# soedinglab/spacedust

Measured on AMD Instinct MI355X. Metric: clustersearch throughput (genome-pairs/s; SW GCUPS alongside), higher is better.
Workload: dtype int16

## Files before the change

### include/spacedust_gpu.h

```cpp
#ifndef SPACEDUST_GPU_H
#define SPACEDUST_GPU_H

#include <stddef.h>
#include <stdint.h>

#ifdef __cplusplus
extern "C" {
#endif

enum {
    SD_OK = 0,
    SD_ENODEVICE = -1,
    SD_EHIP = -2,
    SD_EINVAL = -3,
    SD_ENOMEM = -4,
    SD_EUNSUPPORTED = -5,
    SD_EMISMATCH = -6
};

typedef struct sd_ctx sd_ctx;
typedef struct sd_seqset sd_seqset;
typedef struct sd_target sd_target;

int sd_ctx_create(int device, sd_ctx **out);
// ... 59 lines not shown
                                    uint32_t nPairs, const uint32_t *pairQ, const uint32_t *pairT, const uint16_t *pairDiag,
                                    const uint8_t *isIdentity, float seqIdThr, int32_t alnLenThr, uint32_t *outIdx, sd_sw_result *out,
                                    uint32_t *nOut, char *btPool, uint64_t btCap, uint64_t *btUsed);

int sd_sw_align_alt_batch(sd_ctx *ctx, const sd_sw_params *par, const sd_seqset *queries, const sd_seqset *targets, uint32_t nSeeds,
                          const uint32_t *seedQ, const uint32_t *seedT, const int32_t *tStart, const int32_t *tEnd,
                          const uint8_t *isIdentity, uint32_t maxAlt, float seqIdThr, int32_t alnLenThr, int32_t seqIdMode,
                          sd_sw_result *out, uint32_t *outCount, char *btPool, uint64_t btCap, uint64_t *btUsed);
int sd_sw_alt_last_stats(sd_ctx *ctx, uint64_t *groups, uint64_t *seedRounds, uint64_t *bytesCopied);

int sd_sw_set_cigar_pool(sd_ctx *ctx, int on);
int sd_sw_download_bytes(sd_ctx *ctx, uint64_t *recordBytes, uint64_t *poolBytes);

int sd_sw_set_narrow_final(sd_ctx *ctx, int on);
int sd_sw_set_shared_start(sd_ctx *ctx, int on);

int sd_selftest_sort_pairs(sd_ctx *ctx, const uint32_t *keys, const uint32_t *vals, uint32_t n, int beginBit, int endBit, uint32_t *outKeys,
                           uint32_t *outVals);
int sd_selftest_scan(sd_ctx *ctx, const uint32_t *in, uint32_t n, uint64_t *exclusiveSum, uint32_t *runningMax);
int sd_selftest_score_class(int kernel , int32_t n, int32_t tL, int shared, int32_t wideRowLimit,
                            uint32_t *klass, char *scope, size_t cap);
int sd_selftest_r2p_weights(sd_ctx *ctx, uint32_t nTasks, const uint32_t *nRows, const uint32_t *L, const uint8_t *cells, float *freq,
                            float *eff);
struct sd_kmermatch_params_s;
int sd_selftest_kmermatch_records(sd_ctx *ctx, const struct sd_kmermatch_params_s *par, uint64_t nSeq, const uint8_t *residues,
                                  const uint64_t *offsets, const uint32_t *keys, const uint8_t *letterMap21, uint64_t recCap,
                                  uint32_t *seqConsidered, uint32_t *seqThreshold, uint32_t *seqExcess, uint64_t *recOff, uint64_t *recKey,
                                  uint32_t *recId, uint32_t *recLen, uint32_t *recPos, uint64_t *stats);

int sd_sw_align_batch_hostpath(sd_ctx *ctx, const sd_sw_params *par, const sd_seqset *queries, const sd_seqset *targets,
// ... 430 lines not shown
```

### spacedust_amd/_lib.py

```python
import ctypes as C
import os

import numpy as np

HERE = os.path.dirname(os.path.abspath(__file__))
LIB_PATH = os.path.join(HERE, 'libsdgpu.so')

_vp = C.c_void_p


SD_OK, SD_ENODEVICE, SD_EHIP, SD_EINVAL, SD_ENOMEM, SD_EUNSUPPORTED, SD_EMISMATCH = 0, -1, -2, -3, -4, -5, -6


class SdError(RuntimeError):
    pass


class SwParams(C.Structure):
    _fields_ = [('gapOpen', C.c_int32), ('gapExtend', C.c_int32), ('matrix', C.c_int8 * 441), ('covMode', C.c_int32),
                ('covThr', C.c_float), ('evalThr', C.c_double), ('swMode', C.c_int32), ('dbResidues', C.c_uint64)]


class SwResult(C.Structure):
    _fields_ = [('score', C.c_int32), ('qStart', C.c_int32), ('qEnd', C.c_int32), ('tStart', C.c_int32),
# ... 223 lines not shown
        'sd_search_result_arrays': (C.c_int, [_vp] + [_vp] * 12),
        'sd_search_result_write_tsv': (C.c_int, [_vp, C.c_char_p, C.c_char_p, _vp, C.c_char_p, _vp, C.c_char_p, _vp, C.c_char_p, _vp,
                                                 C.c_int, C.c_int, C.c_uint64, C.POINTER(C.c_uint64), C.POINTER(C.c_uint64)]),
        'sd_search_result_records': (C.c_int, [_vp, _vp, C.c_uint64, C.POINTER(C.c_uint64)]),
        'sd_agg_records': (C.c_int, [_vp] * 7 + [_vp, C.c_uint64, C.POINTER(C.c_uint64)]),
        'sd_records_check': (C.c_int, [_vp, C.c_uint64, C.c_uint32, C.c_uint32, C.c_uint32, C.c_uint32, C.POINTER(C.c_uint64), C.POINTER(C.c_uint64)]),
        'sd_records_write_tsv': (C.c_int, [_vp, C.c_uint64, C.c_char_p, C.c_int, C.c_uint64, C.c_char_p, _vp, C.c_char_p, _vp, C.c_char_p, _vp,
                                           C.c_char_p, _vp, C.c_int, C.POINTER(C.c_uint64), C.POINTER(C.c_uint64)]),
        'sd_search_result_destroy': (None, [_vp]),
        'sd_search_stats': (C.c_int, [_vp, _vp, _vp]),
        'sd_search_download_bytes': (C.c_int, [_vp, C.POINTER(C.c_uint64), C.POINTER(C.c_uint64)]),
        'sd_sw_set_cigar_pool': (C.c_int, [_vp, C.c_int]),
        'sd_sw_download_bytes': (C.c_int, [_vp, C.POINTER(C.c_uint64), C.POINTER(C.c_uint64)]),
        'sd_sw_set_narrow_final': (C.c_int, [_vp, C.c_int]),
        'sd_sw_set_shared_start': (C.c_int, [_vp, C.c_int]),
        'sd_r2p_create': (C.c_int, [C.POINTER(_vp)]),
        'sd_r2p_destroy': (None, [_vp]),
        'sd_r2p_batch': (C.c_int, [_vp, C.POINTER(R2pParams), C.c_uint32] + [_vp] * 12),
        'sd_r2p_batch_device': (C.c_int, [_vp, _vp, C.POINTER(R2pParams), C.c_uint32] + [_vp] * 12),
        'sd_selftest_r2p_weights': (C.c_int, [_vp, C.c_uint32, _vp, _vp, _vp, _vp, _vp]),
        'sd_selftest_score_class': (C.c_int, [C.c_int, C.c_int32, C.c_int32, C.c_int, C.c_int32, C.POINTER(C.c_uint32), C.c_char_p, C.c_size_t]),
        'sd_shard_query_sets': (C.c_int, [_vp, C.c_uint32, C.c_uint32, C.c_uint32, _vp, C.POINTER(C.c_uint32)]),
        'sd_comm_unique_id': (C.c_int, [C.c_char_p]),
        'sd_comm_init': (C.c_int, [C.c_int, C.c_int, C.c_int, C.c_char_p, C.POINTER(_vp)]),
        'sd_comm_destroy': (None, [_vp]),
        'sd_comm_host_buffer': (C.c_int, [_vp, C.c_int, C.c_uint64, C.POINTER(_vp)]),
        'sd_comm_last_error': (C.c_char_p, [_vp]),
        'sd_search_set_records_sink': (C.c_int, [_vp, _vp, _vp]),
        'sd_gather_stream_begin': (C.c_int, [_vp, C.c_int, C.c_uint32, _vp, C.c_uint32, _vp, C.c_uint64, C.c_int, C.POINTER(_vp)]),
        'sd_gather_stream_end': (C.c_int, [_vp, _vp, _vp, C.POINTER(C.c_uint64)]),
# ... 62 lines not shown
```

### spacedust_amd/api.py

```python
import ctypes as C

import numpy as np

from . import _lib
from .cpus import effective_cpus
from ._lib import SdError, ptr


def _check(ctx, rc, what):
    if rc != 0:
        msg = ''
        if ctx is not None:
            msg = _lib.load().sd_last_error(ctx).decode(errors='replace')
        raise SdError('%s failed (%d): %s' % (what, rc, msg))


class Host:

    def __init__(self, threads=0):
        import os
        self.L = _lib.load()
        self.threads = threads or effective_cpus()
        h = C.c_void_p()
        _check(None, self.L.sd_host_create(self.threads, C.byref(h)), 'sd_host_create')
# ... 444 lines not shown
        out = np.zeros(len(hq), _lib.RESCORE_DTYPE)
        _check(self.h, self.L.sd_rescore_diagonal_batch(self.h, C.byref(par), queries.h, targets.h, len(hq), ptr(hq), ptr(ht), ptr(hd),
                                                        ptr(out)), 'sd_rescore_diagonal_batch')
        return out

    def set_cigar_pool(self, on=True):
        _check(self.h, self.L.sd_sw_set_cigar_pool(self.h, 1 if on else 0), 'sd_sw_set_cigar_pool')
        self._cigar_pool = bool(on)

    def set_narrow_final(self, on=True):
        _check(self.h, self.L.sd_sw_set_narrow_final(self.h, 1 if on else 0), 'sd_sw_set_narrow_final')

    def set_shared_start(self, on=True):
        _check(self.h, self.L.sd_sw_set_shared_start(self.h, 1 if on else 0), 'sd_sw_set_shared_start')

    def sw_download_bytes(self):
        a, b = C.c_uint64(), C.c_uint64()
        self.L.sd_sw_download_bytes(self.h, C.byref(a), C.byref(b))
        return a.value, b.value

    def sw_cells(self):
        f, r, t = C.c_uint64(), C.c_uint64(), C.c_uint64()
        self.L.sd_sw_last_cells(self.h, C.byref(f), C.byref(r), C.byref(t))
        return f.value, r.value, t.value

    def __del__(self):
        try:
            h, self.h = self.h, None
            if h:
                self.L.sd_ctx_destroy(h)
# ... 511 lines not shown
```

### spacedust_amd/csrc/cli/sd_mod_iter.cpp

```cpp
#include "sd_align_core.h"
#include "sd_cli.h"
#include "sd_pref_core.h"

#include <algorithm>
#include <atomic>
#include <chrono>
#include <climits>
#include <cmath>
#include <condition_variable>
#include <cstdio>
#include <cstdlib>
#include <cstring>
#include <memory>
#include <mutex>
#include <omp.h>
#include <string>
#include <sys/resource.h>
#include <thread>
#include <vector>

namespace sdcli {

namespace {

// ... 43 lines not shown

struct Worker {
    sd_ctx *ctx = nullptr;
    sd_host *host = nullptr;
    sd_r2p *r2p = nullptr;
    int threads = 1;
    QueryChunk Q;
    std::vector<uint8_t> failed;
    AlignChunk C;
    std::vector<uint32_t> mark;
    uint32_t stamp = 0;
    ~Worker() {
        if (r2p) sd_r2p_destroy(r2p);
        if (ctx) sd_sw_set_narrow_final(ctx, 0);
        if (ctx) sd_sw_set_shared_start(ctx, 0);
        if (ctx) sd_ctx_destroy(ctx);
        if (host) sd_host_destroy(host);
    }
};

double quantE(double v) {
    char text[32];
    double back = v;
    sd_host_quantise_3e(v, text, &back);
    return back;
}

int failChunk(ChunkOut &o, int rc, const std::string &what, sd_ctx *ctx) {
    o.rc = rc;
    o.err = what + " failed (" + std::to_string(rc) + ")";
// ... 255 lines not shown
    nWorkers = std::max(1, std::min(nWorkers, 8));
    uint32_t chunkQ = (uint32_t) std::max<long long>(1, a.integer("--iter-chunk-queries", getenv("SD_ITER_CHUNK") ? atoi(getenv("SD_ITER_CHUNK")) : 1500));
    const int perWorker = std::max(1, std::min(threads, (threads * 3 / 2 + nWorkers - 1) / nWorkers));
    std::vector<std::unique_ptr<Worker> > workers;
    for (int w = 0; w < nWorkers; w++) {
        workers.emplace_back(new Worker());
        Worker &W = *workers.back();
        W.threads = perWorker;
        int rc = sd_ctx_create(device, &W.ctx);
        if (rc != SD_OK) return failNoDevice(rc);
        if (sd_host_create(perWorker, &W.host) != SD_OK) return fail("sd_host_create failed");
        if (sd_r2p_create(&W.r2p) != SD_OK) return fail("sd_r2p_create failed");
        if (S.profile) sd_profile_enable(W.ctx, 1);
        sd_sw_set_narrow_final(W.ctx, (getenv("SD_SW_NARROW_FINAL") && atoi(getenv("SD_SW_NARROW_FINAL")) == 0) ? 0 : 1);
        sd_sw_set_shared_start(W.ctx, (getenv("SD_SW_SHARED_START") && atoi(getenv("SD_SW_SHARED_START")) == 0) ? 0 : 1);
    }
    uint64_t indexEntries = 0;
    TargetH seqTarget, profTarget;
    SeqSetH tset;
    {
        sd_ctx *c0 = workers[0]->ctx;
        uint64_t st[2] = {0, 0};
        if (int rc = buildTarget(host.h, c0, S.pfSeq, tdb->residues.data(), tdb->offsets.data(), tdb->n, &seqTarget.t, st)) return rc;
        indexEntries = st[0];
        info(a, "Index table k-mer threshold: %d at k-mer size %d\nIndex statistics\nEntries:          %llu\n", S.pfSeq.kmerThr, S.pfSeq.k,
             (unsigned long long) st[0]);
        if (numIt > 1) {
            if (int rc = buildTarget(host.h, c0, S.pfProf, tdb->residues.data(), tdb->offsets.data(), tdb->n, &profTarget.t, st, std::string(),
                                     "sd_target_build (profile searches)"))
                return rc;
// ... 420 lines not shown
```

### spacedust_amd/csrc/hip/sd_common.h

```cpp
#ifndef SD_COMMON_H
#define SD_COMMON_H

#include <hip/hip_runtime.h>

#include <cstdarg>
#include <cstdint>
#include <cstdio>
#include <cstring>
#include <algorithm>
#include <ctime>
#include <sys/prctl.h>
#include <map>
#include <mutex>
#include <string>
#include <vector>

#include "spacedust_gpu.h"

struct sd_profile_entry {
    double ms = 0.0;
    uint64_t launches = 0;
};

struct sd_ctx {
    int device = 0;
    hipStream_t stream = nullptr;
    std::string lastError;
    bool profiling = false;
    std::map<std::string, sd_profile_entry> profile;
    hipEvent_t evStart = nullptr, evStop = nullptr;
    bool biasTablesUploaded = false;
    hipEvent_t evSync = nullptr;
    uint64_t cellsFwd = 0, cellsRev = 0, cellsTb = 0;
    uint64_t cellsUngapped = 0;
    uint64_t altGroups = 0, altSeedRounds = 0, altBytes = 0;
    const sd_sw_result *alignDevRes = nullptr;
    size_t alignDevResN = 0;
    bool cigarPool = false;
    bool sharedStart = false;
    bool narrowFinal = false;
    uint64_t d2hRecordBytes = 0, d2hPoolBytes = 0;
    struct ExpandState {
        uint64_t nPairs = 0, runsRead = 0, bytesWritten = 0;
        uint32_t nAB = 0;
        const int32_t *abStartA = nullptr, *abStartB = nullptr, *bcStartB = nullptr, *bcStartC = nullptr;
        const uint64_t *abRunOff = nullptr, *bcRowOff = nullptr, *bcRunOff = nullptr, *pairOff = nullptr;
        const uint32_t *abRuns = nullptr, *bcRuns = nullptr, *abCluster = nullptr;
        const sd_expand_result *res = nullptr;
    } expand;
    hipDeviceProp_t prop;
    struct WsEntry { void *p = nullptr; size_t bytes = 0; };
    std::map<std::string, WsEntry> ws;
    std::map<std::string, WsEntry> pinned;
    struct ProfPending { std::string name; hipEvent_t a = nullptr, b = nullptr; };
// ... 343 lines not shown
```

### spacedust_amd/csrc/hip/sd_sw.hip

```cpp
#include "sd_common.h"
#include <unistd.h>


#include <algorithm>
#include <cmath>
#include <cstring>
#include <memory>
#include <omp.h>
#include <numeric>

#include "../host/sd_host.h"
#include "sd_sw_pk.h"

namespace {

using sdpk::SwTask;
using sdpk::NARROW_EXACT;

template <int RT>
__global__ void __launch_bounds__(64)
sw_score_kernel(const SwTask *__restrict__ tasks, uint32_t nTasks, const uint8_t *__restrict__ qRes,
                const int8_t *__restrict__ qBias, const uint8_t *__restrict__ tRes, const int8_t *__restrict__ mat,
                int go, int ge, int32_t *__restrict__ out, uint2 *__restrict__ boundary,
                const uint32_t *__restrict__ order ,
// ... 673 lines not shown
}

using ScoreLaunch = void (*)(sd_ctx *ctx, const SwTask *dTasks, const uint32_t *dOrder, uint32_t n, const sd_seqset *q, const sd_seqset *t,
                             const int8_t *dMat, int go, int ge, int32_t *dOut, uint2 *dBound);

template <int RT, int LW, bool MULTI, bool WIDE, bool SHARED>
void launchScorePk(sd_ctx *ctx, const SwTask *dTasks, const uint32_t *dOrder, uint32_t n, const sd_seqset *q,
                   const sd_seqset *t, const int8_t *dMat, int go, int ge, int32_t *dOut, uint2 *dBound) {
    if (n == 0) return;
    constexpr uint32_t perWave = 2 * (64 / LW);
    dim3 grid((n + perWave - 1) / perWave), block(64);
    hipLaunchKernelGGL((sdpk::sw_score_pk_kernel<RT, LW, MULTI, WIDE, SHARED>), grid, block, 0, ctx->stream, dTasks, n, q->dRes, q->dBias,
                       t->dRes, dMat, go, ge, dOut, dBound, dOrder, (const int8_t *) q->dProf);
}

template <int RT, bool SHARED, bool START = false>
void launchScorePkAligned(sd_ctx *ctx, const SwTask *dTasks, const uint32_t *dOrder, uint32_t n, const sd_seqset *q, const sd_seqset *t,
                          const int8_t *dMat, int go, int ge, int32_t *dOut, uint2 * ) {
    if (n == 0) return;
    constexpr uint32_t perWave = 4;
    dim3 grid((n + perWave - 1) / perWave), block(64);
    hipLaunchKernelGGL((sdpk::sw_score_pk_aligned_kernel<RT, SHARED, START>), grid, block, 0, ctx->stream, dTasks, n, q->dRes, q->dBias, t->dRes,
                       dMat, go, ge, dOut, dOrder, (const int8_t *) q->dProf);
}

template <int RT>
void launchScoreIdx(sd_ctx *ctx, const SwTask *dTasks, const uint32_t *dOrder, uint32_t n, const sd_seqset *q,
                    const sd_seqset *t, const int8_t *dMat, int go, int ge, int32_t *dOut, uint2 *dBound) {
    if (n == 0) return;
    dim3 grid((n + 1) / 2), block(64);
    hipLaunchKernelGGL(sw_score_kernel<RT>, grid, block, 0, ctx->stream, dTasks, n, q->dRes, q->dBias, t->dRes, dMat,
                       go, ge, dOut, dBound, dOrder, (const int8_t *) q->dProf);
}

enum ScoreKernel { SCORE_PK = 0, SCORE_PK_WIDE = 1, SCORE_INT32 = 2, SCORE_PK_START = 3 };
constexpr int START_ROWS_MIN = 129, START_ROWS_MAX = 768;
// ... 746 lines not shown
    }
    need[i] = v;
}
__global__ void __launch_bounds__(256)
k_bound_apply(uint32_t nPairs, SwTask *__restrict__ tasks, const uint64_t *__restrict__ off) {
    const uint32_t i = blockIdx.x * blockDim.x + threadIdx.x;
    if (i >= nPairs) return;
    tasks[i].boundOff = off[i];
}

constexpr uint32_t PAIR_NONE = 0xFFFFFFFFu;
constexpr int PAIR_QUERY_BITS = 17;
__host__ __device__ __forceinline__ bool pairedClass(uint32_t ci, int startOnly) {
    return startOnly ? ci >= FIRST_START_CLASS && ci < N_SCORE_CLASSES : ci < FIRST_INT32_CLASS;
}
__global__ void __launch_bounds__(256)
k_pair_keys(uint32_t n, const uint32_t *__restrict__ keys, const uint32_t *__restrict__ pairQ, uint32_t *__restrict__ key2, int startOnly) {
    const uint32_t i = blockIdx.x * blockDim.x + threadIdx.x;
    if (i >= n) return;
    const uint32_t k = keys[i];
    uint32_t v = k == KEY_INVALID ? 0xFFFFFFFFu : ((k >> 10) << 26) | (pairQ[i] << 9) | ((k & 1023u) >> 1);
    if (startOnly && k != KEY_INVALID && !pairedClass(k >> 10, startOnly)) v = ((k >> 10) << 26) | ((k & 1023u) << 16);
    key2[i] = v;
}
__global__ void __launch_bounds__(256)
k_pair_heads(uint32_t n, const uint32_t *__restrict__ keyS, uint32_t *__restrict__ headPos) {
    const uint32_t p = blockIdx.x * blockDim.x + threadIdx.x;
    if (p >= n) return;
    const bool head = p == 0 || (keyS[p] >> 9) != (keyS[p - 1] >> 9);
    headPos[p] = head ? p : 0u;
}
__global__ void __launch_bounds__(256)
k_pair_leaders(uint32_t n, const uint32_t *__restrict__ keyS, const uint32_t *__restrict__ runStart, uint8_t *__restrict__ leader,
               int startOnly) {
    const uint32_t p = blockIdx.x * blockDim.x + threadIdx.x;
    if (p > n) return;
    uint8_t v = 0;
    if (p < n && pairedClass(keyS[p] >> 26, startOnly)) {
        const uint32_t o = p - runStart[p];
        v = (o & 1u) == 0 ? 1 : 0;
        const bool lastOfRun = p + 1 >= n || (keyS[p + 1] >> 9) != (keyS[p] >> 9);
        const uint32_t pairs = (o + 1 + 1) / 2;
        if (lastOfRun) v += (uint8_t) (pairs & 1u);
    }
    leader[p] = v;
}
__global__ void __launch_bounds__(256)
k_pair_emit(uint32_t n, const uint32_t *__restrict__ keyS, const uint32_t *__restrict__ vals, const uint32_t *__restrict__ runStartOf,
            const uint64_t *__restrict__ pairIdx, uint32_t *__restrict__ order2, int startOnly) {
    const uint32_t p = blockIdx.x * blockDim.x + threadIdx.x;
    if (p >= n || !pairedClass(keyS[p] >> 26, startOnly) || ((p - runStartOf[p]) & 1u)) return;
    const uint64_t w = pairIdx[p];
    order2[2 * w] = vals[p];
    const bool mate = p + 1 < n && (keyS[p + 1] >> 9) == (keyS[p] >> 9);
    order2[2 * w + 1] = mate ? vals[p + 1] : PAIR_NONE;
}
__global__ void k_pair_bounds(const uint32_t *__restrict__ keyS, uint32_t n, const uint64_t *__restrict__ pairIdx,
                              uint32_t *__restrict__ b, int nb) {
// ... 30 lines not shown
                int startOnly = 0 ) {
    const uint32_t *dOrder = w.dOrder;
    const unsigned grid = (nPairs + 255) / 256;
    int rc = SD_OK;
    uint32_t *dOrder2 = nullptr, *dPairBounds = nullptr;
    if (dPairQ) {
        uint32_t *dKey2 = nullptr, *dVals2 = nullptr, *dHead = nullptr, *dRunStart = nullptr;
        uint64_t *dPairIdx = nullptr;
        uint8_t *dLeader = nullptr;
        SD_HIP(ctx, wsGet(ctx, "sp.key2", (size_t) nPairs, &dKey2));
        SD_HIP(ctx, wsGet(ctx, "sp.vals2", (size_t) nPairs, &dVals2));
        SD_HIP(ctx, wsGet(ctx, "sp.head", (size_t) nPairs, &dHead));
        SD_HIP(ctx, wsGet(ctx, "sp.runstart", (size_t) nPairs, &dRunStart));
        SD_HIP(ctx, wsGet(ctx, "sp.leader", (size_t) nPairs + 1, &dLeader));
        SD_HIP(ctx, wsGet(ctx, "sp.pairidx", (size_t) nPairs + 1, &dPairIdx));
        const size_t order2Cap = (size_t) 4 * nPairs + 8;
        SD_HIP(ctx, wsGet(ctx, "sp.order2", order2Cap, &dOrder2));
        SD_HIP(ctx, hipMemsetAsync(dOrder2, 0xFF, order2Cap * sizeof(uint32_t), ctx->stream));
        SD_HIP(ctx, wsGet(ctx, "sp.bounds", 64, &dPairBounds));
        hipLaunchKernelGGL(k_pair_keys, dim3(grid), dim3(256), 0, ctx->stream, nPairs, dKeys, dPairQ, dKey2, startOnly);
        rc = devSortPairs(ctx, dKey2, w.dKeysS, w.dVals, dVals2, nPairs, 32);
        if (rc != SD_OK) return rc;
        dOrder = dVals2;
        hipLaunchKernelGGL(k_pair_heads, dim3(grid), dim3(256), 0, ctx->stream, nPairs, w.dKeysS, dHead);
        rc = devInclusiveMax(ctx, dHead, dRunStart, nPairs);
        if (rc != SD_OK) return rc;
        hipLaunchKernelGGL(k_pair_leaders, dim3((nPairs + 256) / 256), dim3(256), 0, ctx->stream, nPairs, w.dKeysS, dRunStart, dLeader, startOnly);
        rc = devExclusiveScan(ctx, (const uint8_t *) dLeader, dPairIdx, (size_t) nPairs + 1);
        if (rc != SD_OK) return rc;
        hipLaunchKernelGGL(k_pair_emit, dim3(grid), dim3(256), 0, ctx->stream, nPairs, w.dKeysS, dVals2, dRunStart, dPairIdx, dOrder2, startOnly);
        hipLaunchKernelGGL(k_pair_bounds, dim3(1), dim3(64), 0, ctx->stream, w.dKeysS, nPairs, dPairIdx, dPairBounds,
                           (int) N_SCORE_CLASSES + 1);
        hipLaunchKernelGGL(k_bounds, dim3(1), dim3(64), 0, ctx->stream, w.dKeysS, nPairs, 1u << 26, w.dBounds, (int) N_SCORE_CLASSES + 1);
    } else {
        rc = devSortPairs(ctx, dKeys, w.dKeysS, w.dVals, w.dOrder, nPairs, 16);
        if (rc != SD_OK) return rc;
        hipLaunchKernelGGL(k_bounds, dim3(1), dim3(64), 0, ctx->stream, w.dKeysS, nPairs, 1024u, w.dBounds, (int) N_SCORE_CLASSES + 1);
    }
    hipLaunchKernelGGL(k_bound_need, dim3(grid), dim3(256), 0, ctx->stream, nPairs, w.dTasks, dKeys, w.dScanA);
    SD_HIP(ctx, hipMemsetAsync(w.dScanA + nPairs, 0, sizeof(uint64_t), ctx->stream));
    rc = devExclusiveScan(ctx, w.dScanA, w.dScanB, (size_t) nPairs + 1);
    if (rc != SD_OK) return rc;
// ... 875 lines not shown
int sd_sw_set_cigar_pool(sd_ctx *ctx, int on) {
    if (!ctx) return SD_EINVAL;
    ctx->cigarPool = on != 0;
    return SD_OK;
}

int sd_sw_set_narrow_final(sd_ctx *ctx, int on) {
    if (!ctx) return SD_EINVAL;
    ctx->narrowFinal = on != 0;
    return SD_OK;
}

int sd_sw_set_shared_start(sd_ctx *ctx, int on) {
    if (!ctx) return SD_EINVAL;
    ctx->sharedStart = on != 0;
    return SD_OK;
}

int sd_sw_download_bytes(sd_ctx *ctx, uint64_t *recordBytes, uint64_t *poolBytes) {
    if (!ctx) return SD_EINVAL;
    if (recordBytes) *recordBytes = ctx->d2hRecordBytes;
    if (poolBytes) *poolBytes = ctx->d2hPoolBytes;
    return SD_OK;
}

int sd_sw_align_batch(sd_ctx *ctx, const sd_sw_params *par, const sd_seqset *queries, const sd_seqset *targets,
                      uint32_t nPairs, const uint32_t *pairQ, const uint32_t *pairT, const uint8_t *isIdentity,
                      sd_sw_result *out, char *btPool, uint64_t btCap, uint64_t *btUsed) {
    return alignBatchImpl(ctx, {par, queries, targets, nPairs, pairQ, pairT, isIdentity, out, btPool, btCap, btUsed, nullptr, nullptr, nullptr, nullptr});
}
// ... 308 lines not shown
```

### spacedust_amd/csrc/hip/sd_sw_pk.h

```cpp
#ifndef SD_SW_PK_H
#define SD_SW_PK_H

#include <hip/hip_runtime.h>
#include <cstdint>

namespace sdpk {

struct SwTask {
    uint64_t qOff;
    uint64_t tOff;
    int32_t n;
    int32_t tL;
    int32_t qStep;
    int32_t tStep;
    int32_t segLen;
    uint32_t slot;
    uint64_t boundOff;
};

typedef short s16x2 __attribute__((ext_vector_type(2)));
typedef unsigned short u16x2 __attribute__((ext_vector_type(2)));

__device__ __forceinline__ uint32_t pkMax(uint32_t a, uint32_t b) {
    return __builtin_bit_cast(uint32_t, __builtin_elementwise_max(__builtin_bit_cast(s16x2, a), __builtin_bit_cast(s16x2, b)));
// ... 26 lines not shown
    asm("v_add_u16_sdwa %0, %4, sext(%8) dst_sel:WORD_0 dst_unused:UNUSED_PAD src0_sel:WORD_0 src1_sel:BYTE_0\n\t"
        "v_add_u16_sdwa %1, %5, sext(%8) dst_sel:WORD_0 dst_unused:UNUSED_PAD src0_sel:WORD_0 src1_sel:BYTE_1\n\t"
        "v_add_u16_sdwa %2, %6, sext(%8) dst_sel:WORD_0 dst_unused:UNUSED_PAD src0_sel:WORD_0 src1_sel:BYTE_2\n\t"
        "v_add_u16_sdwa %3, %7, sext(%8) dst_sel:WORD_0 dst_unused:UNUSED_PAD src0_sel:WORD_0 src1_sel:BYTE_3\n\t"
        "v_add_u16_sdwa %0, %4, sext(%9) dst_sel:WORD_1 dst_unused:UNUSED_PRESERVE src0_sel:WORD_1 src1_sel:BYTE_0\n\t"
        "v_add_u16_sdwa %1, %5, sext(%9) dst_sel:WORD_1 dst_unused:UNUSED_PRESERVE src0_sel:WORD_1 src1_sel:BYTE_1\n\t"
        "v_add_u16_sdwa %2, %6, sext(%9) dst_sel:WORD_1 dst_unused:UNUSED_PRESERVE src0_sel:WORD_1 src1_sel:BYTE_2\n\t"
        "v_add_u16_sdwa %3, %7, sext(%9) dst_sel:WORD_1 dst_unused:UNUSED_PRESERVE src0_sel:WORD_1 src1_sel:BYTE_3\n\t"
        "s_nop 0"
        : "=&v"(h0), "=&v"(h1), "=&v"(h2), "=&v"(h3)
        : "v"(d0), "v"(d1), "v"(d2), "v"(d3), "v"(pa), "v"(pb));
}

__device__ __forceinline__ uint32_t dppShr1(uint32_t v) {
    return (uint32_t) __builtin_amdgcn_update_dpp(0, (int) v, 0x138 , 0xf, 0xf, false);
}

template <int LANE>
__device__ __forceinline__ uint32_t writeLane(uint32_t value, uint32_t old) {
    asm("v_writelane_b32 %0, %1, %2" : "+v"(old) : "s"(value), "n"(LANE));
    return old;
}
__device__ __forceinline__ uint32_t readLane(uint32_t v, int lane) {
#if defined(__HIP_DEVICE_COMPILE__)
    return (uint32_t) __builtin_amdgcn_readlane((int) v, lane);
#else
    (void) lane;
    return v;
#endif
}
// ... 267 lines not shown
    uint32_t r;
    asm("v_bfi_b32 %0, %1, %2, %3" : "=v"(r) : "v"(mask), "v"(a), "v"(b));
    return r;
}
__device__ __forceinline__ uint32_t addWord0(uint32_t base, uint32_t packed) {
    uint32_t r;
    asm("v_add_u32_sdwa %0, %1, %2 dst_sel:DWORD dst_unused:UNUSED_PAD src0_sel:DWORD src1_sel:WORD_0" : "=v"(r) : "v"(base), "v"(packed));
    return r;
}
__device__ __forceinline__ uint32_t addWord1(uint32_t base, uint32_t packed) {
    uint32_t r;
    asm("v_add_u32_sdwa %0, %1, %2 dst_sel:DWORD dst_unused:UNUSED_PAD src0_sel:DWORD src1_sel:WORD_1" : "=v"(r) : "v"(base), "v"(packed));
    return r;
}

template <int RT, bool SHARED, bool START = false>
__global__ void __launch_bounds__(64)
sw_score_pk_aligned_kernel(const SwTask *__restrict__ tasks, uint32_t nTasks, const uint8_t *__restrict__ qRes,
                           const int8_t *__restrict__ qBias, const uint8_t *__restrict__ tRes, const int8_t *__restrict__ mat,
                           int go, int ge, int32_t *__restrict__ out, const uint32_t *__restrict__ order,
                           const int8_t *__restrict__ qProf) {
    constexpr int LW = 32;
    constexpr int WORDS = (RT + 3) / 4;
    constexpr int RTP = 4 * WORDS;
    constexpr int PSTRIDE = LW * WORDS;
    constexpr int NGRP = 64 / LW;
    constexpr int NT = 2 * NGRP;
    constexpr uint32_t ROWB = PSTRIDE * 4;
    static_assert(22 * ROWB < 65536, "row offsets travel in 16 bits");
    static_assert(SHARED || !START, "the start-row form has one profile per wavefront");
    __shared__ uint32_t prof[SHARED ? 1 : NT][22][PSTRIDE];
    __shared__ int8_t smat[441];
    for (int i = threadIdx.x; i < 441; i += 64) smat[i] = mat[i];
    __syncthreads();
    const int lane = threadIdx.x & 63, wave = threadIdx.x >> 6;
    const int grp = lane / LW, l = lane % LW;
    SwTask tk[NT];
#pragma unroll
    for (int x = 0; x < NT; x++) {
        const uint32_t id = (blockIdx.x + (uint32_t) wave) * NT + x;
        const uint32_t tid = id < nTasks ? (order ? order[id] : id) : 0xFFFFFFFFu;
        if (tid != 0xFFFFFFFFu) {
            tk[x] = tasks[tid];
        } else {
            tk[x].n = 0; tk[x].tL = 0; tk[x].qOff = 0; tk[x].tOff = 0; tk[x].qStep = 1; tk[x].tStep = 1; tk[x].segLen = START ? 0 : 1;
// ... 8 lines not shown
            B = tk[2 * g + 1];
        }
    const bool haveA = A.n > 0, haveB = B.n > 0;
    if (SHARED && !haveB) {
        B = A;
        B.tL = 0;
    }
    int maxN = 0, maxTL = 0;
#pragma unroll
    for (int x = 0; x < NT; x++) {
        maxN = max(maxN, tk[x].n);
        maxTL = max(maxTL, tk[x].tL);
    }
    const int steps = (maxN > 0 && maxTL > 0) ? maxTL + LW - 1 : 0;
    const uint32_t goP = (uint32_t) go | ((uint32_t) go << 16), geP = (uint32_t) ge | ((uint32_t) ge << 16);
    const int q0 = l * RT;
#pragma unroll
    for (int x = 0; x < (SHARED ? 1 : 2); x++) {
        const SwTask &T = SHARED ? tk[0] : (x ? B : A);
        const int64_t pOff = START ? (int64_t) T.qOff - (int64_t) T.segLen * T.qStep : (int64_t) T.qOff;
        const int pN = START ? T.n + T.segLen : T.n;
        uint32_t *pw = &prof[SHARED ? 0 : 2 * grp + x][0][0] + l * WORDS;
#pragma unroll
        for (int w = 0; w < WORDS; w++) {
            int res[4], cb[4];
            int64_t pidx[4];
            bool valid[4];
#pragma unroll
            for (int b = 0; b < 4; b++) {
                const int qi = q0 + 4 * w + b;
                valid[b] = (4 * w + b < RT) && qi < pN;
                res[b] = 20;
                cb[b] = 0;
                pidx[b] = 0;
                if (valid[b]) {
                    const int64_t idx = pOff + (int64_t) qi * T.qStep;
                    res[b] = qRes[idx];
                    cb[b] = qBias[idx];
                    pidx[b] = idx * 21;
                }
            }
            const int aFirst = SHARED ? wave * NGRP + grp : 0, aStep = SHARED ? NGRP : 1;
            if (qProf) {
                for (int a = aFirst; a < 21; a += aStep) {
                    uint32_t word = 0;
#pragma unroll
// ... 42 lines not shown
            keepA[w] = l != sA ? 0xFFFFFFFFu : (dropA == 4 ? 0u : 0xFFFFFFFFu << (8 * dropA));
            keepB[w] = l != sB ? 0xFFFFFFFFu : (dropB == 4 ? 0u : 0xFFFFFFFFu << (8 * dropB));
        }
    }
    constexpr uint32_t NEUT = (uint32_t) PK_NEUTRAL * ROWB;
    auto loadChunk = [&](int c0) -> uint32_t {
        const int col = c0 + l;
        uint32_t a = PK_NEUTRAL, b = PK_NEUTRAL;
        if (col < A.tL) a = tRes[(int64_t) A.tOff + (int64_t) col * A.tStep];
        if (col < B.tL) b = tRes[(int64_t) B.tOff + (int64_t) col * B.tStep];
        return (a * ROWB) | ((b * ROWB) << 16);
    };
    uint32_t chunk = loadChunk(0);
    uint32_t chunkNext = loadChunk(LW);
    uint32_t T = NEUT | (NEUT << 16);
    T = writeLane<0>(readLane(chunk, 0), T);
    T = writeLane<32>(readLane(chunk, 32), T);
    uint32_t pa[WORDS], pb[WORDS];
    {
        const uint32_t aA = addWord0(baseA, T), aB = addWord1(baseB, T);
#pragma unroll
        for (int w = 0; w < WORDS; w++) {
            pa[w] = ldsWord(aA, w);
            pb[w] = ldsWord(aB, w);
        }
    }
    auto columnStep = [&](const int k, const uint32_t &Tc, const uint32_t (&pac)[WORDS], const uint32_t (&pbc)[WORDS], uint32_t &Tn,
                          uint32_t (&pan)[WORDS], uint32_t (&pbn)[WORDS]) {
        const int i1 = (k + 1) & (LW - 1);
        if (i1 == 0) {
            chunk = chunkNext;
            chunkNext = loadChunk(k + 1 + LW);
        }
        Tn = dppShr1(Tc);
        Tn = writeLane<0>(readLane(chunk, i1), Tn);
        Tn = writeLane<32>(readLane(chunk, 32 + i1), Tn);
        {
            const uint32_t aA = addWord0(baseA, Tn), aB = addWord1(baseB, Tn);
#pragma unroll
            for (int w = 0; w < WORDS; w++) {
                pan[w] = ldsWord(aA, w);
                pbn[w] = ldsWord(aB, w);
            }
        }
        uint32_t inG = dppShr1(outG), inFf = dppShr1(outFf);
        if (START) {
            inG &= handMask;
            inFf &= handMask;
        } else {
            inG = writeLane<32>(0, inG);
            inFf = writeLane<32>(0, inFf);
        }
        uint32_t h[RTP];
#pragma unroll
        for (int w = 0; w < WORDS; w++) {
            const uint32_t d0 = (w == 0) ? prevInG : H[4 * w - 1];
            const uint32_t qa = START ? bfiAsm(keepA[w], pac[w], neutralWord) : pac[w];
            const uint32_t qb = START ? bfiAsm(keepB[w], pbc[w], neutralWord) : pbc[w];
            addProfile4(qa, qb, d0, H[4 * w], H[4 * w + 1], H[4 * w + 2], h[4 * w], h[4 * w + 1], h[4 * w + 2], h[4 * w + 3]);
        }
        prevInG = inG;
        uint32_t Ff = inFf, cm = 0;
#pragma unroll
        for (int r = 0; r < RT; r++) {
            const uint32_t hpre = pkMax(h[r], E[r]);
            const uint32_t g = pkMax(hpre, Ff);
            const uint32_t open = pkSubSat(hpre, goP);
            E[r] = pkMax(pkSubSat(E[r], geP), open);
            Ff = pkMax(pkSubSat(Ff, geP), open);
            H[r] = g;
            const uint32_t code = pkRowCode(g, 31 - r);
            cm = r == 0 ? code : pkMax(cm, code);
        }
        outG = H[RT - 1];
        outFf = Ff;
        const uint32_t t = bestcm | 0x001F001Fu;
        const uint32_t m = pkAshr15(pkSub(t, cm));
        const uint32_t kk = (uint32_t) k | ((uint32_t) k << 16);
        bestcm = bfiAsm(m, cm, bestcm);
        bestcol = bfiAsm(m, kk, bestcol);
    };
    uint32_t T2, pa2[WORDS], pb2[WORDS];
#pragma unroll 1
    for (int k = 0; k < steps; k += 2) {
        columnStep(k, T, pa, pb, T2, pa2, pb2);
        columnStep(k + 1, T2, pa2, pb2, T, pa, pb);
    }
    unsigned long long keyA = 0, keyB = 0;
    {
// ... 32 lines not shown
```

### spacedust_amd/csrc/host/sd_search.cpp

```cpp
#include "sd_host.h"
#include "sd_target_build.h"
#include "spacedust_gpu.h"

#include <algorithm>
#include <chrono>
#include <condition_variable>
#include <cstdio>
#include <cstdlib>
#include <cstring>
#include <deque>
#include <fstream>
#include <functional>
#include <future>
#include <memory>
#include <mutex>
#include <string>
#include <thread>
#include <pthread.h>
#include <vector>

namespace {

double nowSec() {
    return std::chrono::duration<double>(std::chrono::steady_clock::now().time_since_epoch()).count();
// ... 459 lines not shown
            for (sd_ctx *c : al)
                if (c) sd_sw_set_narrow_final(c, 0);
        }
    } narrowFinalMode(s, !(getenv("SD_SW_NARROW_FINAL") && atoi(getenv("SD_SW_NARROW_FINAL")) == 0));
    struct SharedStartMode {
        sd_ctx *al[4];
        explicit SharedStartMode(sd_search *s_, bool on) : al{s_->ctxAl, s_->ctxAl2, s_->ctxAlMore[0], s_->ctxAlMore[1]} {
            for (sd_ctx *c : al)
                if (c) sd_sw_set_shared_start(c, on ? 1 : 0);
        }
        ~SharedStartMode() {
            for (sd_ctx *c : al)
                if (c) sd_sw_set_shared_start(c, 0);
        }
    } sharedStartMode(s, !(getenv("SD_SW_SHARED_START") && atoi(getenv("SD_SW_SHARED_START")) == 0));
    std::vector<uint32_t> qSetSize(Q->nSets, 0);
    if (aggregate)
        for (uint32_t i = 0; i < Q->n; i++)
            if (Q->setId[i] < Q->nSets) qSetSize[Q->setId[i]]++;
    if (aggregate) {
        uint32_t m = 0;
        for (uint32_t v : qSetSize) m = std::max(m, v);
        for (uint32_t v : s->tSetSize) m = std::max(m, v);
        for (uint32_t i = 0; i < Q->n; i++) m = std::max(m, Q->posInSet[i]);
        for (uint32_t i = 0; i < T.n; i++) m = std::max(m, T.posInSet[i]);
        if (s->lgamma.size() < (size_t) m + 8) {
            s->lgamma.resize((size_t) m + 8);
            sd_host_lgamma_table(s->lgamma.data(), (uint32_t) s->lgamma.size());
        }
    }
// ... 586 lines not shown
```

Before: 3044.

## Pack four query-sharing pairs per wavefront using 16-lane DPP-row groups

Adds a group16 mode, on by default, for the shared-profile aligned scoring kernel. For aligned classes up to 448 rows, each 32-lane half-wavefront is split into two 16-lane DPP rows, each handling twice as many rows per lane. A wavefront then processes four pairs sharing one query profile instead of two. Leader padding and order-buffer sizing change so query runs are grouped in multiples of four. The aim is to cut wasted diagonal steps and lane idle time for shorter queries, at the cost of more registers per lane, longer per-lane row loops, and more padding slots.

```diff
diff --git a/include/spacedust_gpu.h b/include/spacedust_gpu.h
--- a/include/spacedust_gpu.h
+++ b/include/spacedust_gpu.h
@@ -97,6 +97,7 @@
 
 int sd_sw_set_narrow_final(sd_ctx *ctx, int on);
 int sd_sw_set_shared_start(sd_ctx *ctx, int on);
+int sd_sw_set_group16(sd_ctx *ctx, int on);
 
 int sd_selftest_sort_pairs(sd_ctx *ctx, const uint32_t *keys, const uint32_t *vals, uint32_t n, int beginBit, int endBit, uint32_t *outKeys,
                            uint32_t *outVals);
diff --git a/spacedust_amd/_lib.py b/spacedust_amd/_lib.py
--- a/spacedust_amd/_lib.py
+++ b/spacedust_amd/_lib.py
@@ -261,6 +261,7 @@
         'sd_sw_download_bytes': (C.c_int, [_vp, C.POINTER(C.c_uint64), C.POINTER(C.c_uint64)]),
         'sd_sw_set_narrow_final': (C.c_int, [_vp, C.c_int]),
         'sd_sw_set_shared_start': (C.c_int, [_vp, C.c_int]),
+        'sd_sw_set_group16': (C.c_int, [_vp, C.c_int]),
         'sd_r2p_create': (C.c_int, [C.POINTER(_vp)]),
         'sd_r2p_destroy': (None, [_vp]),
         'sd_r2p_batch': (C.c_int, [_vp, C.POINTER(R2pParams), C.c_uint32] + [_vp] * 12),
diff --git a/spacedust_amd/api.py b/spacedust_amd/api.py
--- a/spacedust_amd/api.py
+++ b/spacedust_amd/api.py
@@ -482,6 +482,9 @@
     def set_shared_start(self, on=True):
         _check(self.h, self.L.sd_sw_set_shared_start(self.h, 1 if on else 0), 'sd_sw_set_shared_start')
 
+    def set_group16(self, on=True):
+        _check(self.h, self.L.sd_sw_set_group16(self.h, 1 if on else 0), 'sd_sw_set_group16')
+
     def sw_download_bytes(self):
         a, b = C.c_uint64(), C.c_uint64()
         self.L.sd_sw_download_bytes(self.h, C.byref(a), C.byref(b))
diff --git a/spacedust_amd/csrc/cli/sd_mod_iter.cpp b/spacedust_amd/csrc/cli/sd_mod_iter.cpp
--- a/spacedust_amd/csrc/cli/sd_mod_iter.cpp
+++ b/spacedust_amd/csrc/cli/sd_mod_iter.cpp
@@ -81,6 +81,7 @@
         if (r2p) sd_r2p_destroy(r2p);
         if (ctx) sd_sw_set_narrow_final(ctx, 0);
         if (ctx) sd_sw_set_shared_start(ctx, 0);
+        if (ctx) sd_sw_set_group16(ctx, 0);
         if (ctx) sd_ctx_destroy(ctx);
         if (host) sd_host_destroy(host);
     }
@@ -366,6 +367,7 @@
         if (S.profile) sd_profile_enable(W.ctx, 1);
         sd_sw_set_narrow_final(W.ctx, (getenv("SD_SW_NARROW_FINAL") && atoi(getenv("SD_SW_NARROW_FINAL")) == 0) ? 0 : 1);
         sd_sw_set_shared_start(W.ctx, (getenv("SD_SW_SHARED_START") && atoi(getenv("SD_SW_SHARED_START")) == 0) ? 0 : 1);
+        sd_sw_set_group16(W.ctx, (getenv("SD_SW_GROUP16") && atoi(getenv("SD_SW_GROUP16")) == 0) ? 0 : 1);
     }
     uint64_t indexEntries = 0;
     TargetH seqTarget, profTarget;
diff --git a/spacedust_amd/csrc/hip/sd_common.h b/spacedust_amd/csrc/hip/sd_common.h
--- a/spacedust_amd/csrc/hip/sd_common.h
+++ b/spacedust_amd/csrc/hip/sd_common.h
@@ -38,6 +38,7 @@
     size_t alignDevResN = 0;
     bool cigarPool = false;
     bool sharedStart = false;
+    bool group16 = false;
     bool narrowFinal = false;
     uint64_t d2hRecordBytes = 0, d2hPoolBytes = 0;
     struct ExpandState {
diff --git a/spacedust_amd/csrc/hip/sd_sw.hip b/spacedust_amd/csrc/hip/sd_sw.hip
--- a/spacedust_amd/csrc/hip/sd_sw.hip
+++ b/spacedust_amd/csrc/hip/sd_sw.hip
@@ -711,12 +711,23 @@
                        t->dRes, dMat, go, ge, dOut, dBound, dOrder, (const int8_t *) q->dProf);
 }
 
+constexpr int GROUP16_ROWS_MAX = 448;
+constexpr __host__ __device__ uint32_t pairsPerWave(uint32_t ci, int startOnly, int group16);
+constexpr uint32_t alignedClass(int RT) { return (uint32_t) RT - 4; }
+
 template <int RT, bool SHARED, bool START = false>
 void launchScorePkAligned(sd_ctx *ctx, const SwTask *dTasks, const uint32_t *dOrder, uint32_t n, const sd_seqset *q, const sd_seqset *t,
                           const int8_t *dMat, int go, int ge, int32_t *dOut, uint2 * ) {
     if (n == 0) return;
-    constexpr uint32_t perWave = 4;
+    const uint32_t perWave = (SHARED && !START) ? 2 * pairsPerWave(alignedClass(RT), 0, ctx->group16 ? 1 : 0) : 4;
     dim3 grid((n + perWave - 1) / perWave), block(64);
+    if constexpr (SHARED && !START && 32 * RT <= GROUP16_ROWS_MAX) {
+        if (perWave == 8) {
+            hipLaunchKernelGGL((sdpk::sw_score_pk_aligned_kernel<RT, true, false, 16>), grid, block, 0, ctx->stream, dTasks, n, q->dRes, q->dBias,
+                               t->dRes, dMat, go, ge, dOut, dOrder, (const int8_t *) q->dProf);
+            return;
+        }
+    }
     hipLaunchKernelGGL((sdpk::sw_score_pk_aligned_kernel<RT, SHARED, START>), grid, block, 0, ctx->stream, dTasks, n, q->dRes, q->dBias, t->dRes,
                        dMat, go, ge, dOut, dOrder, (const int8_t *) q->dProf);
 }
@@ -1493,6 +1504,12 @@
 __host__ __device__ __forceinline__ bool pairedClass(uint32_t ci, int startOnly) {
     return startOnly ? ci >= FIRST_START_CLASS && ci < N_SCORE_CLASSES : ci < FIRST_INT32_CLASS;
 }
+constexpr __host__ __device__ uint32_t pairsPerWave(uint32_t ci, int startOnly, int group16) {
+    return group16 && !startOnly && ci >= alignedClass(5) && ci <= alignedClass(GROUP16_ROWS_MAX / 32) ? 4u : 2u;
+}
+static_assert(SCORE_CLASSES[alignedClass(5)].form == SCORE_PK && SCORE_CLASSES[alignedClass(5)].rows == 5 * 32 &&
+              SCORE_CLASSES[alignedClass(24)].form == SCORE_PK && SCORE_CLASSES[alignedClass(24)].rows == 24 * 32,
+              "alignedClass: a_seg5 .. a_seg24 are the classes 1 .. 20");
 __global__ void __launch_bounds__(256)
 k_pair_keys(uint32_t n, const uint32_t *__restrict__ keys, const uint32_t *__restrict__ pairQ, uint32_t *__restrict__ key2, int startOnly) {
     const uint32_t i = blockIdx.x * blockDim.x + threadIdx.x;
@@ -1511,7 +1528,7 @@
 }
 __global__ void __launch_bounds__(256)
 k_pair_leaders(uint32_t n, const uint32_t *__restrict__ keyS, const uint32_t *__restrict__ runStart, uint8_t *__restrict__ leader,
-               int startOnly) {
+               int startOnly, int group16) {
     const uint32_t p = blockIdx.x * blockDim.x + threadIdx.x;
     if (p > n) return;
     uint8_t v = 0;
@@ -1520,7 +1537,8 @@
         v = (o & 1u) == 0 ? 1 : 0;
         const bool lastOfRun = p + 1 >= n || (keyS[p + 1] >> 9) != (keyS[p] >> 9);
         const uint32_t pairs = (o + 1 + 1) / 2;
-        if (lastOfRun) v += (uint8_t) (pairs & 1u);
+        const uint32_t ppw = pairsPerWave(keyS[p] >> 26, startOnly, group16);
+        if (lastOfRun) v += (uint8_t) ((ppw - pairs % ppw) % ppw);
     }
     leader[p] = v;
 }
@@ -1581,7 +1599,7 @@
         SD_HIP(ctx, wsGet(ctx, "sp.runstart", (size_t) nPairs, &dRunStart));
         SD_HIP(ctx, wsGet(ctx, "sp.leader", (size_t) nPairs + 1, &dLeader));
         SD_HIP(ctx, wsGet(ctx, "sp.pairidx", (size_t) nPairs + 1, &dPairIdx));
-        const size_t order2Cap = (size_t) 4 * nPairs + 8;
+        const size_t order2Cap = (size_t) 8 * nPairs + 16;
         SD_HIP(ctx, wsGet(ctx, "sp.order2", order2Cap, &dOrder2));
         SD_HIP(ctx, hipMemsetAsync(dOrder2, 0xFF, order2Cap * sizeof(uint32_t), ctx->stream));
         SD_HIP(ctx, wsGet(ctx, "sp.bounds", 64, &dPairBounds));
@@ -1592,7 +1610,8 @@
         hipLaunchKernelGGL(k_pair_heads, dim3(grid), dim3(256), 0, ctx->stream, nPairs, w.dKeysS, dHead);
         rc = devInclusiveMax(ctx, dHead, dRunStart, nPairs);
         if (rc != SD_OK) return rc;
-        hipLaunchKernelGGL(k_pair_leaders, dim3((nPairs + 256) / 256), dim3(256), 0, ctx->stream, nPairs, w.dKeysS, dRunStart, dLeader, startOnly);
+        hipLaunchKernelGGL(k_pair_leaders, dim3((nPairs + 256) / 256), dim3(256), 0, ctx->stream, nPairs, w.dKeysS, dRunStart, dLeader, startOnly,
+                           ctx->group16 ? 1 : 0);
         rc = devExclusiveScan(ctx, (const uint8_t *) dLeader, dPairIdx, (size_t) nPairs + 1);
         if (rc != SD_OK) return rc;
         hipLaunchKernelGGL(k_pair_emit, dim3(grid), dim3(256), 0, ctx->stream, nPairs, w.dKeysS, dVals2, dRunStart, dPairIdx, dOrder2, startOnly);
@@ -2498,6 +2517,12 @@
 int sd_sw_set_shared_start(sd_ctx *ctx, int on) {
     if (!ctx) return SD_EINVAL;
     ctx->sharedStart = on != 0;
+    return SD_OK;
+}
+
+int sd_sw_set_group16(sd_ctx *ctx, int on) {
+    if (!ctx) return SD_EINVAL;
+    ctx->group16 = on != 0;
     return SD_OK;
 }
 
diff --git a/spacedust_amd/csrc/hip/sd_sw_pk.h b/spacedust_amd/csrc/hip/sd_sw_pk.h
--- a/spacedust_amd/csrc/hip/sd_sw_pk.h
+++ b/spacedust_amd/csrc/hip/sd_sw_pk.h
@@ -64,6 +64,16 @@
 
 __device__ __forceinline__ uint32_t dppShr1(uint32_t v) {
     return (uint32_t) __builtin_amdgcn_update_dpp(0, (int) v, 0x138 , 0xf, 0xf, false);
+}
+
+__device__ __forceinline__ uint32_t dppRowShr1(uint32_t v) {
+    return (uint32_t) __builtin_amdgcn_update_dpp(0, (int) v, 0x111 , 0xf, 0xf, true);
+}
+__device__ __forceinline__ uint32_t dppRowShr1Keep(uint32_t first, uint32_t v) {
+    return (uint32_t) __builtin_amdgcn_update_dpp((int) first, (int) v, 0x111 , 0xf, 0xf, false);
+}
+__device__ __forceinline__ uint32_t dppRowRol1(uint32_t v) {
+    return (uint32_t) __builtin_amdgcn_update_dpp(0, (int) v, 0x12F , 0xf, 0xf, false);
 }
 
 template <int LANE>
@@ -361,21 +371,24 @@
     return r;
 }
 
-template <int RT, bool SHARED, bool START = false>
+template <int RT, bool SHARED, bool START = false, int LW = 32>
 __global__ void __launch_bounds__(64)
 sw_score_pk_aligned_kernel(const SwTask *__restrict__ tasks, uint32_t nTasks, const uint8_t *__restrict__ qRes,
                            const int8_t *__restrict__ qBias, const uint8_t *__restrict__ tRes, const int8_t *__restrict__ mat,
                            int go, int ge, int32_t *__restrict__ out, const uint32_t *__restrict__ order,
                            const int8_t *__restrict__ qProf) {
-    constexpr int LW = 32;
-    constexpr int WORDS = (RT + 3) / 4;
+    constexpr int RTL = RT * (32 / LW);
+    constexpr int WORDS = (RTL + 3) / 4;
     constexpr int RTP = 4 * WORDS;
     constexpr int PSTRIDE = LW * WORDS;
     constexpr int NGRP = 64 / LW;
     constexpr int NT = 2 * NGRP;
     constexpr uint32_t ROWB = PSTRIDE * 4;
+    static_assert(LW == 32 || LW == 16, "a group is half a wavefront or one DPP row");
     static_assert(22 * ROWB < 65536, "row offsets travel in 16 bits");
     static_assert(SHARED || !START, "the start-row form has one profile per wavefront");
+    static_assert(LW == 32 || (SHARED && !START), "16-lane groups: the shared forward form only");
+    static_assert(RTL <= 32, "the row code has five row bits: 16-lane groups end at RT = 16 (512 rows), a_seg17 .. a_seg24 stay on 32 lanes");
     __shared__ uint32_t prof[SHARED ? 1 : NT][22][PSTRIDE];
     __shared__ int8_t smat[441];
     for (int i = threadIdx.x; i < 441; i += 64) smat[i] = mat[i];
@@ -414,7 +427,7 @@
     }
     const int steps = (maxN > 0 && maxTL > 0) ? maxTL + LW - 1 : 0;
     const uint32_t goP = (uint32_t) go | ((uint32_t) go << 16), geP = (uint32_t) ge | ((uint32_t) ge << 16);
-    const int q0 = l * RT;
+    const int q0 = l * RTL;
 #pragma unroll
     for (int x = 0; x < (SHARED ? 1 : 2); x++) {
         const SwTask &T = SHARED ? tk[0] : (x ? B : A);
@@ -429,7 +442,7 @@
 #pragma unroll
             for (int b = 0; b < 4; b++) {
                 const int qi = q0 + 4 * w + b;
-                valid[b] = (4 * w + b < RT) && qi < pN;
+                valid[b] = (4 * w + b < RTL) && qi < pN;
                 res[b] = 20;
                 cb[b] = 0;
                 pidx[b] = 0;
@@ -502,8 +515,12 @@
     uint32_t chunk = loadChunk(0);
     uint32_t chunkNext = loadChunk(LW);
     uint32_t T = NEUT | (NEUT << 16);
-    T = writeLane<0>(readLane(chunk, 0), T);
-    T = writeLane<32>(readLane(chunk, 32), T);
+    if (LW == 32) {
+        T = writeLane<0>(readLane(chunk, 0), T);
+        T = writeLane<32>(readLane(chunk, 32), T);
+    } else {
+        T = l == 0 ? chunk : T;
+    }
     uint32_t pa[WORDS], pb[WORDS];
     {
         const uint32_t aA = addWord0(baseA, T), aB = addWord1(baseB, T);
@@ -519,10 +536,16 @@
         if (i1 == 0) {
             chunk = chunkNext;
             chunkNext = loadChunk(k + 1 + LW);
-        }
-        Tn = dppShr1(Tc);
-        Tn = writeLane<0>(readLane(chunk, i1), Tn);
-        Tn = writeLane<32>(readLane(chunk, 32 + i1), Tn);
+        } else if (LW == 16) {
+            chunk = dppRowRol1(chunk);
+        }
+        if (LW == 32) {
+            Tn = dppShr1(Tc);
+            Tn = writeLane<0>(readLane(chunk, i1), Tn);
+            Tn = writeLane<32>(readLane(chunk, 32 + i1), Tn);
+        } else {
+            Tn = dppRowShr1Keep(chunk, Tc);
+        }
         {
             const uint32_t aA = addWord0(baseA, Tn), aB = addWord1(baseB, Tn);
 #pragma unroll
@@ -531,11 +554,11 @@
                 pbn[w] = ldsWord(aB, w);
             }
         }
-        uint32_t inG = dppShr1(outG), inFf = dppShr1(outFf);
+        uint32_t inG = LW == 32 ? dppShr1(outG) : dppRowShr1(outG), inFf = LW == 32 ? dppShr1(outFf) : dppRowShr1(outFf);
         if (START) {
             inG &= handMask;
             inFf &= handMask;
-        } else {
+        } else if (LW == 32) {
             inG = writeLane<32>(0, inG);
             inFf = writeLane<32>(0, inFf);
         }
@@ -550,7 +573,7 @@
         prevInG = inG;
         uint32_t Ff = inFf, cm = 0;
 #pragma unroll
-        for (int r = 0; r < RT; r++) {
+        for (int r = 0; r < RTL; r++) {
             const uint32_t hpre = pkMax(h[r], E[r]);
             const uint32_t g = pkMax(hpre, Ff);
             const uint32_t open = pkSubSat(hpre, goP);
@@ -560,7 +583,7 @@
             const uint32_t code = pkRowCode(g, 31 - r);
             cm = r == 0 ? code : pkMax(cm, code);
         }
-        outG = H[RT - 1];
+        outG = H[RTL - 1];
         outFf = Ff;
         const uint32_t t = bestcm | 0x001F001Fu;
         const uint32_t m = pkAshr15(pkSub(t, cm));
diff --git a/spacedust_amd/csrc/host/sd_search.cpp b/spacedust_amd/csrc/host/sd_search.cpp
--- a/spacedust_amd/csrc/host/sd_search.cpp
+++ b/spacedust_amd/csrc/host/sd_search.cpp
@@ -497,6 +497,17 @@
                 if (c) sd_sw_set_shared_start(c, 0);
         }
     } sharedStartMode(s, !(getenv("SD_SW_SHARED_START") && atoi(getenv("SD_SW_SHARED_START")) == 0));
+    struct Group16Mode {
+        sd_ctx *al[4];
+        explicit Group16Mode(sd_search *s_, bool on) : al{s_->ctxAl, s_->ctxAl2, s_->ctxAlMore[0], s_->ctxAlMore[1]} {
+            for (sd_ctx *c : al)
+                if (c) sd_sw_set_group16(c, on ? 1 : 0);
+        }
+        ~Group16Mode() {
+            for (sd_ctx *c : al)
+                if (c) sd_sw_set_group16(c, 0);
+        }
+    } group16Mode(s, !(getenv("SD_SW_GROUP16") && atoi(getenv("SD_SW_GROUP16")) == 0));
     std::vector<uint32_t> qSetSize(Q->nSets, 0);
     if (aggregate)
         for (uint32_t i = 0; i < Q->n; i++)
```

After: 3164 (median of 6 runs). +3.9%, better.
